# vccheng2001/DeepVCP-Pointcloud-Registration

Hardware: AMD Instinct MI355X
Metric: pairs/sec (full DeepVCP forward) at N=16384, K=64; rot/trans error vs ref (higher is better)
Workload: dtype f32

## Files before the change

### deepvcp-pointcloud-registration_amd/csrc/sa_mlp_mfma.hip

```cpp
#include "common.h"
#include "morton.h"

namespace dvcp {

typedef float f32x16 __attribute__((ext_vector_type(16)));
typedef __bf16 bf16x8 __attribute__((ext_vector_type(8)));

#ifndef DVCP_SA_SPLIT3
#define DVCP_SA_SPLIT3 1
#endif
#ifndef DVCP_SA_PACK16
#define DVCP_SA_PACK16 1
#endif

struct Split3 {
  bf16x8 p0, p1, p2;
};
__device__ __forceinline__ Split3 split3(const float (&x)[8]) {
  Split3 s;
#pragma unroll
  for (int j = 0; j < 8; ++j) {
    const __bf16 b0 = static_cast<__bf16>(x[j]);
    const float r1 = x[j] - static_cast<float>(b0);
    const __bf16 b1 = static_cast<__bf16>(r1);
    const float r2 = r1 - static_cast<float>(b1);
    s.p0[j] = b0;
    s.p1[j] = b1;
    s.p2[j] = static_cast<__bf16>(r2);
  }
  return s;
}
__device__ __forceinline__ f32x16 mfma_split3(const Split3& a, const bf16x8& b0, const bf16x8& b1, const bf16x8& b2,
                                             f32x16 acc) {
  acc = __builtin_amdgcn_mfma_f32_32x32x16_bf16(a.p2, b0, acc, 0, 0, 0);
  acc = __builtin_amdgcn_mfma_f32_32x32x16_bf16(a.p1, b1, acc, 0, 0, 0);
  acc = __builtin_amdgcn_mfma_f32_32x32x16_bf16(a.p0, b2, acc, 0, 0, 0);
  acc = __builtin_amdgcn_mfma_f32_32x32x16_bf16(a.p1, b0, acc, 0, 0, 0);
  acc = __builtin_amdgcn_mfma_f32_32x32x16_bf16(a.p0, b1, acc, 0, 0, 0);
  return __builtin_amdgcn_mfma_f32_32x32x16_bf16(a.p0, b0, acc, 0, 0, 0);
}

constexpr int kMfmaWaves = 4;

template <int D, int C1, int C2>
struct SaMfmaShape {
  static constexpr int C0 = 3 + D;
  static constexpr int KS = 3 + D / 2;
  static constexpr int MT = C1 / 32;
  static constexpr int CT = C2 / 32;
  static constexpr int K2 = MT * 16;
  static constexpr int KB = MT * 2;
  static_assert(D % 8 == 0 && C1 % 32 == 0 && C2 % 32 == 0, "MFMA tiling");
};

template <int D, int C1, int C2, bool PRE>
struct SaMfmaLds {
  using S = SaMfmaShape<D, C1, C2>;
  float w1[PRE ? 1 : S::MT][S::KS][64];
  float wx[S::MT][2][64];
#if DVCP_SA_SPLIT3
  bf16x8 w2s[S::CT][S::KB][3][64];
#else
  float w2[S::CT][S::K2][64];
#endif
  float b1[S::MT][2][16];
  float s1[S::MT][2][16];
  float t1[S::MT][2][16];
};

template <int D>
__device__ __forceinline__ int sa_in_channel(int s, int h) {
  if (s < 3) return h == 0 ? s : -1;
  return 3 + h * (D / 2) + (s - 3);
}

__device__ __forceinline__ int acc_row(int r, int h) { return (r & 3) + 8 * (r >> 2) + 4 * h; }

template <int D, int C1>
__global__ __launch_bounds__(256) void sa_pre_mfma_kernel(const float* __restrict__ feat, int64_t fb, int64_t fn, int N,
                                                          int B, const float* __restrict__ params,
                                                          float* __restrict__ U, const int64_t* __restrict__ rows,
                                                          int Nf) {
  constexpr int C0 = 3 + D, MT = C1 / 32, KS = D / 2;
  static_assert(D % 8 == 0 && C1 % 32 == 0, "MFMA tiling");
  __shared__ float wf[MT][KS][64];
  __shared__ float bias[C1];
  const float* W1 = params;
  const float* pb1 = W1 + C1 * C0;
  const float* ps1 = pb1 + C1;
  const float* pt1 = ps1 + C1;
  for (int i = threadIdx.x; i < MT * KS * 64; i += blockDim.x) {
    const int l = i % 64, s = (i / 64) % KS, mt = i / (64 * KS), o = 32 * mt + (l & 31);
    wf[mt][s][l] = W1[o * C0 + 3 + s + (l >> 5) * (D / 2)] * ps1[o];
  }
  for (int c = threadIdx.x; c < C1; c += blockDim.x)
    bias[c] = static_cast<float>(static_cast<double>(pb1[c]) * ps1[c] + static_cast<double>(pt1[c]));
  __syncthreads();
  const int lane = threadIdx.x & 63, h = lane >> 5, r32 = lane & 31;
  const int64_t total = static_cast<int64_t>(B) * N;
  const int64_t ntiles = (total + 31) / 32;
  for (int64_t t = static_cast<int64_t>(blockIdx.x) * 4 + (threadIdx.x >> 6); t < ntiles;
       t += static_cast<int64_t>(gridDim.x) * 4) {
    const int64_t i = t * 32 + r32;
    const int64_t ic = i < total ? i : total - 1;
    const int b = static_cast<int>(ic / N), n = static_cast<int>(ic % N);
    int64_t src = n;
    if (rows) {
      const int64_t r = rows[ic];
      src = r < 0 ? 0 : (r >= Nf ? Nf - 1 : r);
    }
    const float4* fr = reinterpret_cast<const float4*>(feat + b * fb + src * fn + h * (D / 2));
    float x[KS];
#pragma unroll
    for (int v = 0; v < KS / 4; ++v) {
      const float4 q = fr[v];
      x[4 * v] = q.x;
      x[4 * v + 1] = q.y;
      x[4 * v + 2] = q.z;
      x[4 * v + 3] = q.w;
    }
    int zo = 0;
    asm volatile("" : "+v"(zo));
    f32x16 acc[MT];
#pragma unroll
    for (int mt = 0; mt < MT; ++mt) {
      const float bc = bias[32 * mt + r32 + zo];
#pragma unroll
      for (int r = 0; r < 16; ++r) acc[mt][r] = bc;
    }
#pragma unroll
    for (int s = 0; s < KS; ++s)
#pragma unroll
      for (int mt = 0; mt < MT; ++mt)
        acc[mt] = __builtin_amdgcn_mfma_f32_32x32x2f32(x[s], wf[mt][s][lane + zo], acc[mt], 0, 0, 0);
#pragma unroll
    for (int r = 0; r < 16; ++r) {
      const int64_t ip = t * 32 + acc_row(r, h);
      if (ip < total)
#pragma unroll
        for (int mt = 0; mt < MT; ++mt) U[ip * C1 + 32 * mt + r32] = acc[mt][r];
    }
  }
}

template <typename T>
__global__ __launch_bounds__(kBuildThreads) void sa_order_kernel(PointsView<T> ctr, int S, int32_t* __restrict__ order) {
  __shared__ uint32_t bins[kSortBins];
  __shared__ uint32_t wsum[16];
  __shared__ float red[2][3][16];
  const int b = blockIdx.x;
  auto get = [&](int i, float (&v)[3]) {
#pragma unroll
    for (int a = 0; a < 3; ++a) v[a] = static_cast<float>(ctr.at(b, a, i));
  };
  float lo[3], hi[3];
  block_bbox(S, get, lo, hi, red);
  int32_t* o = order + static_cast<int64_t>(b) * S;
  morton_sort(S, get, [&](int pos, int i, const float (&)[3]) { o[pos] = i; }, lo, hi, bins, wsum);
}

template <typename T, int D, int C1, int C2, bool PRE, bool PACK = false>
__global__ __launch_bounds__(kMfmaWaves * kWave) __attribute__((amdgpu_waves_per_eu(3))) void sa_mlp_mfma_kernel(
    PointsView<T> pts, PointsView<T> ctr, int S, int B, const float* __restrict__ feat, int64_t fb, int64_t fn,
    const int32_t* __restrict__ count, const int32_t* __restrict__ list, int nsample,
    const float* __restrict__ params, const float* __restrict__ U, int64_t ub, const int32_t* __restrict__ order,
    float* __restrict__ out, int xcd) {
  using Sh = SaMfmaShape<D, C1, C2>;
  constexpr int C0 = Sh::C0, KS = Sh::KS, MT = Sh::MT, CT = Sh::CT;
  __shared__ SaMfmaLds<D, C1, C2, PRE> L;
  const int tid = threadIdx.x, lane = tid & 63, wave = tid >> 6, h = lane >> 5, r32 = lane & 31;

  const float* W1 = params;
  const float* pb1 = W1 + C1 * C0;
  const float* ps1 = pb1 + C1;
  const float* pt1 = ps1 + C1;
  const float* W2 = pt1 + C1;
  const float* pb2 = W2 + C2 * C1;
  const float* ps2 = pb2 + C2;
  const float* pt2 = ps2 + C2;
  if (!PRE)
    for (int i = tid; i < MT * KS * 64; i += blockDim.x) {
      const int l = i % 64, s = (i / 64) % KS, mt = i / (64 * KS);
      const int ch = sa_in_channel<D>(s, l >> 5);
      L.w1[mt][s][l] = ch < 0 ? 0.0f : W1[(32 * mt + (l & 31)) * C0 + ch];
    }
  if (PRE)
    for (int i = tid; i < MT * 2 * 64; i += blockDim.x) {
      const int l = i % 64, s = (i / 64) % 2, mt = i / 128;
      const int ch = s == 0 ? (l >> 5) : ((l >> 5) == 0 ? 2 : -1);
      L.wx[mt][s][l] = ch < 0 ? 0.0f : W1[(32 * mt + (l & 31)) * C0 + ch] * ps1[32 * mt + (l & 31)];
    }
#if DVCP_SA_SPLIT3
  for (int i = tid; i < CT * Sh::KB * 64; i += blockDim.x) {
    const int l = i % 64, s = (i / 64) % Sh::KB, ct = i / (64 * Sh::KB);
    const int o = 32 * ct + (l & 31);
    float w[8];
#pragma unroll
    for (int j = 0; j < 8; ++j)
      w[j] = W2[o * C1 + 32 * (s / 2) + acc_row(8 * (s % 2) + j, l >> 5)] * (PRE ? ps2[o] : 1.0f);
    const Split3 ws = split3(w);
    L.w2s[ct][s][0][l] = ws.p0;
    L.w2s[ct][s][1][l] = ws.p1;
    L.w2s[ct][s][2][l] = ws.p2;
  }
#else
  for (int i = tid; i < CT * Sh::K2 * 64; i += blockDim.x) {
    const int l = i % 64, kk = (i / 64) % Sh::K2, ct = i / (64 * Sh::K2);
    const int mt = kk / 16, r = kk % 16;
    L.w2[ct][kk][l] = W2[(32 * ct + (l & 31)) * C1 + 32 * mt + acc_row(r, l >> 5)] * (PRE ? ps2[32 * ct + (l & 31)] : 1.0f);
  }
#endif
  for (int i = tid; i < MT * 32; i += blockDim.x) {
    const int r = i % 16, hh = (i / 16) % 2, mt = i / 32;
    const int c = 32 * mt + acc_row(r, hh);
    L.b1[mt][hh][r] = pb1[c];
    L.s1[mt][hh][r] = ps1[c];
    L.t1[mt][hh][r] = pt1[c];
  }
  float b2[CT], s2[CT], t2[CT];
#pragma unroll
  for (int ct = 0; ct < CT; ++ct) {
    b2[ct] = pb2[32 * ct + r32];
    s2[ct] = ps2[32 * ct + r32];
    t2[ct] = pt2[32 * ct + r32];
    if (PRE) b2[ct] = static_cast<float>(static_cast<double>(b2[ct]) * s2[ct] + static_cast<double>(t2[ct]));
  }
  __syncthreads();

  int64_t total, q0, qs;
  int xo = 0;
  if (xcd) {
    xo = static_cast<int>(blockIdx.x) & 7;
    total = static_cast<int64_t>((B - xo + 7) / 8) * S;
    q0 = static_cast<int64_t>(blockIdx.x >> 3) * kMfmaWaves + wave;
    qs = static_cast<int64_t>(gridDim.x >> 3) * kMfmaWaves;
  } else {
    total = static_cast<int64_t>(B) * S;
    q0 = static_cast<int64_t>(blockIdx.x) * kMfmaWaves + wave;
    qs = static_cast<int64_t>(gridDim.x) * kMfmaWaves;
  }
  auto lane_bcast = [](auto v, int j) {
    if constexpr (sizeof(v) == 8) {
      const int64_t u = __builtin_bit_cast(int64_t, v);
      const int lo = __builtin_amdgcn_readlane(static_cast<int>(u & 0xFFFFFFFF), j);
      const int hi = __builtin_amdgcn_readlane(static_cast<int>(u >> 32), j);
      return __builtin_bit_cast(decltype(v), (static_cast<int64_t>(hi) << 32) | static_cast<uint32_t>(lo));
    } else {
      return __builtin_bit_cast(decltype(v), __builtin_amdgcn_readlane(__builtin_bit_cast(int, v), j));
    }
  };
  for (int64_t qc = q0; qc < total; qc += 64 * qs) {
    const int64_t qm = qc + lane * qs;
    int m_b = 0, m_rows = 0;
    int64_t m_fc = 0;
    T m_cx = T(0), m_cy = T(0), m_cz = T(0);
    if (qm < total) {
      const int64_t q = xcd ? (xo + 8 * (qm / S)) * static_cast<int64_t>(S) + qm % S : qm;
      m_b = static_cast<int>(q / S);
      const int c = order ? order[q] : static_cast<int>(q % S);
      m_fc = static_cast<int64_t>(m_b) * S + c;
      const int r = count[m_fc];
      m_rows = r < 1 ? 0 : (r > nsample ? nsample : r);
      ctr.load3(m_b, c, m_cx, m_cy, m_cz);
    }
    const int ncen = static_cast<int>(min<int64_t>(64, (total - qc + qs - 1) / qs));
    auto list_entry = [&](int j, int n0) {
      const int64_t fcj = lane_bcast(m_fc, j);
      const int rj = lane_bcast(m_rows, j);
      const int row = n0 + r32;
      return rj == 0 ? 0 : list[fcj * nsample + (row < rj ? row : 0)];
    };
    constexpr bool BZ = PRE && DVCP_SA_SPLIT3;
    if constexpr (PACK) {
      static_assert(!PACK || (PRE && DVCP_SA_SPLIT3), "row packing runs on the split-3 pre-pass path");
      int js = 0, hs = 0;
      auto nh_of = [&](int jj) { return max(1, (lane_bcast(m_rows, jj) + 15) >> 4); };
      int nhj = ncen > 0 ? nh_of(0) : 0;
      int runj = -1;
      float run[CT];
#pragma unroll
      for (int ct = 0; ct < CT; ++ct) run[ct] = 0.0f;
      auto flush = [&]() {
        const int64_t fcr = lane_bcast(m_fc, runj);
        const bool empty = lane_bcast(m_rows, runj) == 0;
#pragma unroll
        for (int ct = 0; ct < CT; ++ct)
          if (h == 0) out[fcr * C2 + 32 * ct + r32] = empty ? 0.0f : fmaxf(run[ct] + b2[ct], 0.0f);
      };
      auto fold = [&](int jj, const float (&m)[CT]) {
        if (jj != runj) {
          if (runj >= 0) flush();
          runj = jj;
#pragma unroll
          for (int ct = 0; ct < CT; ++ct) run[ct] = m[ct];
        } else {
#pragma unroll
          for (int ct = 0; ct < CT; ++ct) run[ct] = fmaxf(run[ct], m[ct]);
        }
      };
      while (js < ncen) {
        const int jA = js, hA = hs;
        if (++hs >= nhj) {
          hs = 0;
          if (++js < ncen) nhj = nh_of(js);
        }
        const bool hasB = js < ncen;
        const int jB = hasB ? js : jA, hB = hasB ? hs : hA;
        if (hasB && ++hs >= nhj) {
          hs = 0;
          if (++js < ncen) nhj = nh_of(js);
        }
        int zo = 0;
        asm volatile("" : "+v"(zo));
        const bool sB = r32 >= 16;
        const int b = sB ? lane_bcast(m_b, jB) : lane_bcast(m_b, jA);
        const int64_t fc = sB ? lane_bcast(m_fc, jB) : lane_bcast(m_fc, jA);
        const int rows = sB ? lane_bcast(m_rows, jB) : lane_bcast(m_rows, jA);
        const T cx = sB ? lane_bcast(m_cx, jB) : lane_bcast(m_cx, jA);
        const T cy = sB ? lane_bcast(m_cy, jB) : lane_bcast(m_cy, jA);
        const T cz = sB ? lane_bcast(m_cz, jB) : lane_bcast(m_cz, jA);
        const int row = 16 * (sB ? hB : hA) + (r32 & 15);
        const int n = rows == 0 ? 0 : list[fc * nsample + (row < rows ? row : 0)];
        f32x16 acc1[MT];
        const float4* ur = reinterpret_cast<const float4*>(U + b * ub + static_cast<int64_t>(n) * C1 + 4 * h);
#pragma unroll
        for (int mt = 0; mt < MT; ++mt)
#pragma unroll
          for (int i = 0; i < 4; ++i) {
            const float4 u = ur[8 * mt + 2 * i];
            acc1[mt][4 * i] = u.x;
            acc1[mt][4 * i + 1] = u.y;
            acc1[mt][4 * i + 2] = u.z;
            acc1[mt][4 * i + 3] = u.w;
          }
        T px, py, pz;
        pts.load3(b, n, px, py, pz);
        const float dx = static_cast<float>(px - cx);
        const float dy = static_cast<float>(py - cy);
        const float dz = static_cast<float>(pz - cz);
        const float x0 = h == 0 ? dx : dy, x1 = h == 0 ? dz : 0.0f;
#pragma unroll
        for (int mt = 0; mt < MT; ++mt) {
          acc1[mt] = __builtin_amdgcn_mfma_f32_32x32x2f32(L.wx[mt][0][lane + zo], x0, acc1[mt], 0, 0, 0);
          acc1[mt] = __builtin_amdgcn_mfma_f32_32x32x2f32(L.wx[mt][1][lane + zo], x1, acc1[mt], 0, 0, 0);
#pragma unroll
          for (int r = 0; r < 16; ++r) acc1[mt][r] = acc1[mt][r] > 0.0f ? acc1[mt][r] : 0.0f;
        }
        f32x16 acc2[CT];
#pragma unroll
        for (int ct = 0; ct < CT; ++ct)
#pragma unroll
          for (int r = 0; r < 16; ++r) acc2[ct][r] = 0.0f;
#pragma unroll
        for (int st = 0; st < Sh::KB; ++st) {
          float x[8];
#pragma unroll
          for (int jj = 0; jj < 8; ++jj) x[jj] = acc1[st / 2][8 * (st % 2) + jj];
          const Split3 a = split3(x);
#pragma unroll
          for (int ct = 0; ct < CT; ++ct)
            acc2[ct] = mfma_split3(a, L.w2s[ct][st][0][lane + zo], L.w2s[ct][st][1][lane + zo],
                                   L.w2s[ct][st][2][lane + zo], acc2[ct]);
        }
        float mA[CT], mB[CT];
#pragma unroll
        for (int ct = 0; ct < CT; ++ct) {
          float a0 = acc2[ct][0], a1 = acc2[ct][8];
#pragma unroll
          for (int r = 1; r < 8; ++r) {
            a0 = fmaxf(a0, acc2[ct][r]);
            a1 = fmaxf(a1, acc2[ct][8 + r]);
          }
          mA[ct] = fmaxf(a0, __shfl_xor(a0, 32, kWave));
          mB[ct] = fmaxf(a1, __shfl_xor(a1, 32, kWave));
        }
        fold(jA, mA);
        if (hasB) fold(jB, mB);
      }
      if (runj >= 0) flush();
      continue;
    }
    const uint64_t live_c = __ballot(lane < ncen && m_rows > 0);
    auto next_live = [&](int j) {
      const uint64_t m = j >= 63 ? 0ull : (live_c & (~0ull << (j + 1)));
      return m ? static_cast<int>(__builtin_ctzll(m)) : 64;
    };
    int n_next = 0;
    {
      const int j0 = (live_c & 1ull) ? 0 : next_live(0);
      if (j0 < ncen) n_next = list_entry(j0, 0);
    }
  for (int j = 0; j < ncen; ++j) {
    const int b = lane_bcast(m_b, j);
    const int64_t fc = lane_bcast(m_fc, j);
    const int rows = lane_bcast(m_rows, j);
    const T cx = lane_bcast(m_cx, j), cy = lane_bcast(m_cy, j), cz = lane_bcast(m_cz, j);
    float mx[CT];
#pragma unroll
    for (int ct = 0; ct < CT; ++ct) mx[ct] = BZ ? -__builtin_huge_valf() : 0.0f;

    for (int n0 = 0; n0 < rows; n0 += 32) {
      int zo = 0;
      asm volatile("" : "+v"(zo));
      const int n = n_next;
      if (n0 + 32 < rows)
        n_next = list_entry(j, n0 + 32);
      else if (next_live(j) < ncen)
        n_next = list_entry(next_live(j), 0);
      f32x16 acc1[MT];
      if constexpr (PRE) {
        const float4* ur = reinterpret_cast<const float4*>(U + b * ub + static_cast<int64_t>(n) * C1 + 4 * h);
#pragma unroll
        for (int mt = 0; mt < MT; ++mt)
#pragma unroll
          for (int i = 0; i < 4; ++i) {
            const float4 u = ur[8 * mt + 2 * i];
            acc1[mt][4 * i] = u.x;
            acc1[mt][4 * i + 1] = u.y;
            acc1[mt][4 * i + 2] = u.z;
            acc1[mt][4 * i + 3] = u.w;
          }
        T px, py, pz;
        pts.load3(b, n, px, py, pz);
        const float dx = static_cast<float>(px - cx);
        const float dy = static_cast<float>(py - cy);
        const float dz = static_cast<float>(pz - cz);
        const float x0 = h == 0 ? dx : dy, x1 = h == 0 ? dz : 0.0f;
#pragma unroll
        for (int mt = 0; mt < MT; ++mt) {
          acc1[mt] = __builtin_amdgcn_mfma_f32_32x32x2f32(L.wx[mt][0][lane + zo], x0, acc1[mt], 0, 0, 0);
          acc1[mt] = __builtin_amdgcn_mfma_f32_32x32x2f32(L.wx[mt][1][lane + zo], x1, acc1[mt], 0, 0, 0);
        }
      } else {
        float x[KS];
        if (h == 0) {
          x[0] = static_cast<float>(pts.at(b, 0, n) - cx);
          x[1] = static_cast<float>(pts.at(b, 1, n) - cy);
          x[2] = static_cast<float>(pts.at(b, 2, n) - cz);
        } else {
          x[0] = x[1] = x[2] = 0.0f;
        }
        const float4* fr = reinterpret_cast<const float4*>(feat + b * fb + static_cast<int64_t>(n) * fn + h * (D / 2));
#pragma unroll
        for (int v = 0; v < D / 8; ++v) {
          const float4 f = fr[v];
          x[3 + 4 * v] = f.x;
          x[4 + 4 * v] = f.y;
          x[5 + 4 * v] = f.z;
          x[6 + 4 * v] = f.w;
        }
#pragma unroll
        for (int mt = 0; mt < MT; ++mt)
#pragma unroll
          for (int r = 0; r < 16; ++r) acc1[mt][r] = L.b1[mt][h][r + zo];
#pragma unroll
        for (int s = 0; s < KS; ++s)
#pragma unroll
          for (int mt = 0; mt < MT; ++mt)
            acc1[mt] = __builtin_amdgcn_mfma_f32_32x32x2f32(L.w1[mt][s][lane + zo], x[s], acc1[mt], 0, 0, 0);
      }
#pragma unroll
      for (int mt = 0; mt < MT; ++mt)
#pragma unroll
        for (int r = 0; r < 16; ++r) {
          const float v = PRE ? acc1[mt][r] : acc1[mt][r] * L.s1[mt][h][r + zo] + L.t1[mt][h][r + zo];
          acc1[mt][r] = v > 0.0f ? v : 0.0f;
        }
      f32x16 acc2[CT];
#pragma unroll
      for (int ct = 0; ct < CT; ++ct)
#pragma unroll
        for (int r = 0; r < 16; ++r) acc2[ct][r] = BZ ? 0.0f : b2[ct];
#if DVCP_SA_SPLIT3
#pragma unroll
      for (int s = 0; s < Sh::KB; ++s) {
        float x[8];
#pragma unroll
        for (int j = 0; j < 8; ++j) x[j] = acc1[s / 2][8 * (s % 2) + j];
        const Split3 a = split3(x);
#pragma unroll
        for (int ct = 0; ct < CT; ++ct)
          acc2[ct] = mfma_split3(a, L.w2s[ct][s][0][lane + zo], L.w2s[ct][s][1][lane + zo], L.w2s[ct][s][2][lane + zo],
                                 acc2[ct]);
      }
#else
#pragma unroll
      for (int mt = 0; mt < MT; ++mt)
#pragma unroll
        for (int r = 0; r < 16; ++r)
#pragma unroll
          for (int ct = 0; ct < CT; ++ct)
            acc2[ct] = __builtin_amdgcn_mfma_f32_32x32x2f32(acc1[mt][r], L.w2[ct][mt * 16 + r][lane + zo], acc2[ct], 0, 0, 0);
#endif
#pragma unroll
      for (int ct = 0; ct < CT; ++ct)
#pragma unroll
        for (int r = 0; r < 16; ++r) {
          if (PRE) {
            mx[ct] = fmaxf(mx[ct], acc2[ct][r]);
          } else {
            const float v = acc2[ct][r] * s2[ct] + t2[ct];
            mx[ct] = fmaxf(mx[ct], v > 0.0f ? v : 0.0f);
          }
        }
    }
#pragma unroll
    for (int ct = 0; ct < CT; ++ct) {
      float m = fmaxf(mx[ct], __shfl_xor(mx[ct], 32, kWave));
      if (BZ) m = fmaxf(m + b2[ct], 0.0f);
      if (h == 0) out[fc * C2 + 32 * ct + r32] = m;
    }
  }
  }
}

struct Sa3Lds {
  float w1[3][64];
  bf16x8 w2[3][64];
  bf16x8 w3[3][64];
  float b1[2][8];
  float b2[2][8];
};

template <typename T, typename FT, int D>
__global__ __launch_bounds__(kMfmaWaves * kWave) void sa3_mfma_kernel(
    PointsView<T> pts, PointsView<T> ctr, int S, int B, const FT* __restrict__ feat, int64_t fb, int64_t fd, int64_t fn,
    const int32_t* __restrict__ count, const int32_t* __restrict__ list, int nsample, const float* __restrict__ params,
    float* __restrict__ out, int xcd) {
  constexpr int C0 = 3 + D, C1 = 16, C2 = 16, C3 = 32;
  constexpr int KS = (C0 + 1) / 2;
  static_assert(D == 0 || D == 3, "sa1 tables");
  __shared__ Sa3Lds L;
  const int tid = threadIdx.x, lane = tid & 63, wave = tid >> 6, h = lane >> 5, r32 = lane & 31;
  const float* W1 = params;
  const float* pb1 = W1 + C1 * C0;
  const float* ps1 = pb1 + C1;
  const float* pt1 = ps1 + C1;
  const float* W2 = pt1 + C1;
  const float* pb2 = W2 + C2 * C1;
  const float* ps2 = pb2 + C2;
  const float* pt2 = ps2 + C2;
  const float* W3 = pt2 + C2;
  const float* pb3 = W3 + C3 * C2;
  const float* ps3 = pb3 + C3;
  const float* pt3 = ps3 + C3;
  auto fold_bias = [](float b, float s, float t) {
    return static_cast<float>(static_cast<double>(b) * s + static_cast<double>(t));
  };
  for (int i = tid; i < KS * 64; i += blockDim.x) {
    const int l = i % 64, s = i / 64, o = l & 31, c = 2 * s + (l >> 5);
    L.w1[s][l] = (o < C1 && c < C0) ? W1[o * C0 + c] * ps1[o] : 0.0f;
  }
  if (tid < 64) {
    const int o = tid & 31, kh = tid >> 5;
    float a[8], w[8];
#pragma unroll
    for (int r = 0; r < 8; ++r) {
      a[r] = o < C2 ? W2[o * C1 + acc_row(r, kh)] * ps2[o] : 0.0f;
      w[r] = W3[o * C2 + acc_row(r, kh)] * ps3[o];
    }
    const Split3 sa = split3(a), sw = split3(w);
    L.w2[0][tid] = sa.p0;
    L.w2[1][tid] = sa.p1;
    L.w2[2][tid] = sa.p2;
    L.w3[0][tid] = sw.p0;
    L.w3[1][tid] = sw.p1;
    L.w3[2][tid] = sw.p2;
  } else if (tid < 80) {
    const int kh = (tid - 64) >> 3, r = tid & 7, c = acc_row(r, kh);
    L.b1[kh][r] = fold_bias(pb1[c], ps1[c], pt1[c]);
    L.b2[kh][r] = fold_bias(pb2[c], ps2[c], pt2[c]);
  }
  const float b3 = fold_bias(pb3[r32], ps3[r32], pt3[r32]);
  __syncthreads();

  int64_t total, q0, qs;
  int xo = 0;
  if (xcd) {
    xo = static_cast<int>(blockIdx.x) & 7;
    total = static_cast<int64_t>((B - xo + 7) / 8) * S;
    q0 = static_cast<int64_t>(blockIdx.x >> 3) * kMfmaWaves + wave;
    qs = static_cast<int64_t>(gridDim.x >> 3) * kMfmaWaves;
  } else {
    total = static_cast<int64_t>(B) * S;
    q0 = static_cast<int64_t>(blockIdx.x) * kMfmaWaves + wave;
    qs = static_cast<int64_t>(gridDim.x) * kMfmaWaves;
  }
  auto lane_bcast = [](auto v, int j) {
    if constexpr (sizeof(v) == 8) {
      const int64_t u = __builtin_bit_cast(int64_t, v);
      const int lo = __builtin_amdgcn_readlane(static_cast<int>(u & 0xFFFFFFFF), j);
      const int hi = __builtin_amdgcn_readlane(static_cast<int>(u >> 32), j);
      return __builtin_bit_cast(decltype(v), (static_cast<int64_t>(hi) << 32) | static_cast<uint32_t>(lo));
    } else {
      return __builtin_bit_cast(decltype(v), __builtin_amdgcn_readlane(__builtin_bit_cast(int, v), j));
    }
  };
  for (int64_t qc = q0; qc < total; qc += 64 * qs) {
    const int64_t qm = qc + lane * qs;
    int m_b = 0, m_rows = 0;
    int64_t m_fc = 0;
    T m_cx = T(0), m_cy = T(0), m_cz = T(0);
    if (qm < total) {
      const int64_t q = xcd ? (xo + 8 * (qm / S)) * static_cast<int64_t>(S) + qm % S : qm;
      m_b = static_cast<int>(q / S);
      m_fc = q;
      const int r = count[q];
      m_rows = r < 0 ? 0 : (r > nsample ? nsample : r);
      const int c = static_cast<int>(q % S);
      ctr.load3(m_b, c, m_cx, m_cy, m_cz);
    }
    const int ncen = static_cast<int>(min<int64_t>(64, (total - qc + qs - 1) / qs));
    int js = 0, hs = 0;
    auto nh_of = [&](int jj) { return max(1, (lane_bcast(m_rows, jj) + 15) >> 4); };
    int nhj = ncen > 0 ? nh_of(0) : 0;
    int runj = -1;
    float run = 0.0f;
    auto flush = [&]() {
      const int64_t fcr = lane_bcast(m_fc, runj);
      const bool empty = lane_bcast(m_rows, runj) == 0;
      if (h == 0) out[fcr * C3 + r32] = empty ? 0.0f : fmaxf(run + b3, 0.0f);
    };
    auto fold = [&](int jj, float m) {
      if (jj != runj) {
        if (runj >= 0) flush();
        runj = jj;
        run = m;
      } else {
        run = fmaxf(run, m);
      }
    };
    while (js < ncen) {
      const int jA = js, hA = hs;
      if (++hs >= nhj) {
        hs = 0;
        if (++js < ncen) nhj = nh_of(js);
      }
      const bool hasB = js < ncen;
      const int jB = hasB ? js : jA, hB = hasB ? hs : hA;
      if (hasB && ++hs >= nhj) {
        hs = 0;
        if (++js < ncen) nhj = nh_of(js);
      }
      int zo = 0;
      asm volatile("" : "+v"(zo));
      const bool sB = r32 >= 16;
      const int b = sB ? lane_bcast(m_b, jB) : lane_bcast(m_b, jA);
      const int64_t fc = sB ? lane_bcast(m_fc, jB) : lane_bcast(m_fc, jA);
      const int rows = sB ? lane_bcast(m_rows, jB) : lane_bcast(m_rows, jA);
      const T cx = sB ? lane_bcast(m_cx, jB) : lane_bcast(m_cx, jA);
      const T cy = sB ? lane_bcast(m_cy, jB) : lane_bcast(m_cy, jA);
      const T cz = sB ? lane_bcast(m_cz, jB) : lane_bcast(m_cz, jA);
      const int row = 16 * (sB ? hB : hA) + (r32 & 15);
      const int n = rows == 0 ? 0 : list[fc * nsample + (row < rows ? row : 0)];
      T px, py, pz;
      pts.load3(b, n, px, py, pz);
      const float dx = static_cast<float>(px - cx);
      const float dy = static_cast<float>(py - cy);
      const float dz = static_cast<float>(pz - cz);
      float x[KS];
      x[0] = h == 0 ? dx : dy;
      if constexpr (D == 0) {
        x[1] = h == 0 ? dz : 0.0f;
      } else {
        const FT* f = feat + b * fb + static_cast<int64_t>(n) * fn;
        x[1] = h == 0 ? dz : static_cast<float>(f[0]);
        x[2] = static_cast<float>(h == 0 ? f[fd] : f[2 * fd]);
      }
      f32x16 a1;
#pragma unroll
      for (int r = 0; r < 8; ++r) {
        a1[r] = L.b1[h][r + zo];
        a1[8 + r] = 0.0f;
      }
#pragma unroll
      for (int s = 0; s < KS; ++s) a1 = __builtin_amdgcn_mfma_f32_32x32x2f32(L.w1[s][lane + zo], x[s], a1, 0, 0, 0);
      float v[8];
#pragma unroll
      for (int r = 0; r < 8; ++r) v[r] = fmaxf(a1[r], 0.0f);
      const Split3 p1 = split3(v);
      f32x16 a2;
#pragma unroll
      for (int r = 0; r < 8; ++r) {
        a2[r] = L.b2[h][r + zo];
        a2[8 + r] = 0.0f;
      }
      const Split3 w2{L.w2[0][lane + zo], L.w2[1][lane + zo], L.w2[2][lane + zo]};
      a2 = mfma_split3(w2, p1.p0, p1.p1, p1.p2, a2);
#pragma unroll
      for (int r = 0; r < 8; ++r) v[r] = fmaxf(a2[r], 0.0f);
      const Split3 p2 = split3(v);
      f32x16 a3;
#pragma unroll
      for (int r = 0; r < 16; ++r) a3[r] = 0.0f;
      a3 = mfma_split3(p2, L.w3[0][lane + zo], L.w3[1][lane + zo], L.w3[2][lane + zo], a3);
      float mA = a3[0], mB = a3[8];
#pragma unroll
      for (int r = 1; r < 8; ++r) {
        mA = fmaxf(mA, a3[r]);
        mB = fmaxf(mB, a3[8 + r]);
      }
      mA = fmaxf(mA, __shfl_xor(mA, 32, kWave));
      mB = fmaxf(mB, __shfl_xor(mB, 32, kWave));
      fold(jA, mA);
      if (hasB) fold(jB, mB);
    }
    if (runj >= 0) flush();
  }
}

#ifndef DVCP_SA_GRID
#define DVCP_SA_GRID 4096
#endif
constexpr int kSaGrid = DVCP_SA_GRID;

template <typename T, typename FT, int D>
int launch_sa3_mfma(const void* xyz, int64_t sb, int64_t sc, int64_t sn, const void* c, int64_t cb, int64_t cc,
                    int64_t cn, int S, int B, const void* feat, int64_t fb, int64_t fd, int64_t fn, const int32_t* count,
                    const int32_t* list, int nsample, const float* params, float* out, hipStream_t st) {
  PointsView<T> pv{static_cast<const T*>(xyz), sb, sc, sn};
  PointsView<T> cv{static_cast<const T*>(c), cb, cc, cn};
  const int64_t centres = static_cast<int64_t>(B) * S;
  const int grid = static_cast<int>(centres < kSaGrid * kMfmaWaves ? (centres + kMfmaWaves - 1) / kMfmaWaves : kSaGrid);
  const int xcd = B % 8 == 0 && grid % 8 == 0 ? 1 : 0;
  hipLaunchKernelGGL((sa3_mfma_kernel<T, FT, D>), dim3(grid), dim3(kMfmaWaves * kWave), 0, st, pv, cv, S, B,
                     static_cast<const FT*>(feat), fb, fd, fn, count, list, nsample, params, out, xcd);
  return launch_status("dvcp_sa_group_mlp(mfma3)");
}

#define DVCP_SA3_MFMA_INST(T, FT, D)                                                                              \
  template int launch_sa3_mfma<T, FT, D>(const void*, int64_t, int64_t, int64_t, const void*, int64_t, int64_t,  \
                                         int64_t, int, int, const void*, int64_t, int64_t, int64_t, const int32_t*, \
                                         const int32_t*, int, const float*, float*, hipStream_t);
DVCP_SA3_MFMA_INST(float, float, 0)
DVCP_SA3_MFMA_INST(float, double, 0)
DVCP_SA3_MFMA_INST(double, float, 0)
DVCP_SA3_MFMA_INST(double, double, 0)
DVCP_SA3_MFMA_INST(float, float, 3)
DVCP_SA3_MFMA_INST(float, double, 3)
DVCP_SA3_MFMA_INST(double, float, 3)
DVCP_SA3_MFMA_INST(double, double, 3)
#undef DVCP_SA3_MFMA_INST

template <typename T, int D, int C1, int C2>
int launch_sa_mfma(const void* xyz, int64_t sb, int64_t sc, int64_t sn, int N, const void* c, int64_t cb, int64_t cc,
                   int64_t cn, int S, int B, const float* feat, int64_t fb, int64_t fn, const int32_t* count,
                   const int32_t* list, int nsample, const float* params, float* U, int32_t* order, float* out,
                   const int64_t* frows, int Nf, hipStream_t st) {
  PointsView<T> pv{static_cast<const T*>(xyz), sb, sc, sn};
  PointsView<T> cv{static_cast<const T*>(c), cb, cc, cn};
  const int64_t centres = static_cast<int64_t>(B) * S;
  const int grid = static_cast<int>(centres < kSaGrid * kMfmaWaves ? (centres + kMfmaWaves - 1) / kMfmaWaves : kSaGrid);
  const int xcd = B % 8 == 0 && grid % 8 == 0 ? 1 : 0;
  if (order)
    hipLaunchKernelGGL((sa_order_kernel<T>), dim3(B), dim3(kBuildThreads), 0, st, cv, S, order);
  if (U) {
    const int64_t rows = static_cast<int64_t>(B) * N;
    const int64_t wgs = (rows + 127) / 128;
    hipLaunchKernelGGL((sa_pre_mfma_kernel<D, C1>), dim3(static_cast<unsigned>(wgs < 2048 ? wgs : 2048)), dim3(256), 0,
                       st, feat, fb, fn, N, B, params, U, frows, Nf);
    if constexpr (DVCP_SA_PACK16 && DVCP_SA_SPLIT3 && D == 32)
      hipLaunchKernelGGL((sa_mlp_mfma_kernel<T, D, C1, C2, true, DVCP_SA_PACK16 && DVCP_SA_SPLIT3>), dim3(grid),
                         dim3(kMfmaWaves * kWave), 0, st, pv, cv, S, B, feat, fb, fn, count, list, nsample, params, U,
                         static_cast<int64_t>(N) * C1, order, out, xcd);
    else
      hipLaunchKernelGGL((sa_mlp_mfma_kernel<T, D, C1, C2, true>), dim3(grid), dim3(kMfmaWaves * kWave), 0, st, pv, cv,
                         S, B, feat, fb, fn, count, list, nsample, params, U, static_cast<int64_t>(N) * C1, order, out, xcd);
  } else {
    hipLaunchKernelGGL((sa_mlp_mfma_kernel<T, D, C1, C2, false>), dim3(grid), dim3(kMfmaWaves * kWave), 0, st, pv,
                       cv, S, B, feat, fb, fn, count, list, nsample, params, nullptr, 0, order, out, xcd);
  }
  return launch_status("dvcp_sa_group_mlp(mfma)");
}

#define DVCP_SA_MFMA_INST(T, D, C1, C2)                                                                          \
  template int launch_sa_mfma<T, D, C1, C2>(const void*, int64_t, int64_t, int64_t, int, const void*, int64_t,  \
                                            int64_t, int64_t, int, int, const float*, int64_t, int64_t,         \
                                            const int32_t*, const int32_t*, int, const float*, float*,          \
                                            int32_t*, float*, const int64_t*, int, hipStream_t);
DVCP_SA_MFMA_INST(float, 32, 32, 64)
DVCP_SA_MFMA_INST(double, 32, 32, 64)
DVCP_SA_MFMA_INST(float, 64, 64, 64)
DVCP_SA_MFMA_INST(double, 64, 64, 64)
#undef DVCP_SA_MFMA_INST

}
```

Baseline: 2523.

## Software-pipeline neighbor loads and interleave split-3 conversion with MFMA in SA kernel

Restructures the SA MLP MFMA kernel so the next tile's neighbor index is fetched one step ahead and its feature and point loads are issued before the current tile's math. It adds a layer-2 helper that computes the bf16 split-3 of the next k-step while the current k-step's MFMAs run, using sched_group_barrier hints to interleave VALU work with MFMA. The non-packed path is flattened into one loop over live center tiles, and empty centers are zero-filled up front. The sa3 kernel also gets a waves_per_eu(4) occupancy hint. The cost is more register pressure from prefetched operands and double-buffered split values, plus more complex control flow.

```diff
diff --git a/deepvcp-pointcloud-registration_amd/csrc/sa_mlp_mfma.hip b/deepvcp-pointcloud-registration_amd/csrc/sa_mlp_mfma.hip
--- a/deepvcp-pointcloud-registration_amd/csrc/sa_mlp_mfma.hip
+++ b/deepvcp-pointcloud-registration_amd/csrc/sa_mlp_mfma.hip
@@ -38,6 +38,78 @@
   acc = __builtin_amdgcn_mfma_f32_32x32x16_bf16(a.p1, b0, acc, 0, 0, 0);
   acc = __builtin_amdgcn_mfma_f32_32x32x16_bf16(a.p0, b1, acc, 0, 0, 0);
   return __builtin_amdgcn_mfma_f32_32x32x16_bf16(a.p0, b0, acc, 0, 0, 0);
+}
+
+constexpr int kSchedValu = 0x2, kSchedMfma = 0x8;
+
+template <int MT, int CT, bool IL>
+__device__ __forceinline__ void sa_layer2_split3(const f32x16 (&acc1)[MT], const bf16x8 (&w2s)[CT][2 * MT][3][64],
+                                                 int li, f32x16 (&acc2)[CT]) {
+  constexpr int KB = 2 * MT;
+  static_assert(CT % 2 == 0, "6 CT MFMAs per k-step in four equal runs");
+  constexpr int Q = 6 * CT / 4;
+  constexpr int VPG = (13 + Q - 1) / Q;
+  auto split_pair = [&](int s, int i, bf16x8 (&p)[3]) {
+#pragma unroll
+    for (int j = 2 * i; j < 2 * i + 2; ++j) {
+      const float v = acc1[s / 2][8 * (s % 2) + j];
+      const float x = v > 0.0f ? v : 0.0f;
+      const __bf16 b0 = static_cast<__bf16>(x);
+      const float r1 = x - static_cast<float>(b0);
+      const __bf16 b1 = static_cast<__bf16>(r1);
+      const float r2 = r1 - static_cast<float>(b1);
+      p[0][j] = b0;
+      p[1][j] = b1;
+      p[2][j] = static_cast<__bf16>(r2);
+    }
+  };
+  if constexpr (!IL) {
+#pragma unroll
+    for (int s = 0; s < KB; ++s) {
+      float x[8];
+#pragma unroll
+      for (int j = 0; j < 8; ++j) {
+        const float v = acc1[s / 2][8 * (s % 2) + j];
+        x[j] = v > 0.0f ? v : 0.0f;
+      }
+      const Split3 as = split3(x);
+#pragma unroll
+      for (int ct = 0; ct < CT; ++ct) acc2[ct] = mfma_split3(as, w2s[ct][s][0][li], w2s[ct][s][1][li], w2s[ct][s][2][li], acc2[ct]);
+    }
+    return;
+  }
+  bf16x8 a[3], an[3];
+#pragma unroll
+  for (int i = 0; i < 4; ++i) split_pair(0, i, a);
+#pragma unroll
+  for (int s = 0; s < KB; ++s) {
+    bf16x8 w[CT][3];
+#pragma unroll
+    for (int ct = 0; ct < CT; ++ct)
+#pragma unroll
+      for (int p = 0; p < 3; ++p) w[ct][p] = w2s[ct][s][p][li];
+#pragma unroll
+    for (int r = 0; r < 4; ++r) {
+      if (s + 1 < KB) split_pair(s + 1, r, an);
+#pragma unroll
+      for (int m = r * Q; m < (r + 1) * Q; ++m) {
+        const int pc = m / CT, ct = m % CT;
+        const int ia = pc == 0 ? 2 : (pc == 1 || pc == 3) ? 1 : 0;
+        const int ib = pc == 2 ? 2 : (pc == 1 || pc == 4) ? 1 : 0;
+        acc2[ct] = __builtin_amdgcn_mfma_f32_32x32x16_bf16(a[ia], w[ct][ib], acc2[ct], 0, 0, 0);
+      }
+      if (s + 1 < KB) {
+#pragma unroll
+        for (int g = 0; g < Q; ++g) {
+          __builtin_amdgcn_sched_group_barrier(kSchedMfma, 1, 0);
+          __builtin_amdgcn_sched_group_barrier(kSchedValu, VPG, 0);
+        }
+      }
+      __builtin_amdgcn_sched_barrier(0);
+    }
+#pragma unroll
+    for (int p = 0; p < 3; ++p) a[p] = an[p];
+  }
 }
 
 constexpr int kMfmaWaves = 4;
@@ -271,6 +343,62 @@
       return rj == 0 ? 0 : list[fcj * nsample + (row < rj ? row : 0)];
     };
     constexpr bool BZ = PRE && DVCP_SA_SPLIT3;
+    constexpr int NV = PRE ? 4 * MT : D / 8;
+    struct Ops {
+      float4 v[NV];
+      T px, py, pz;
+    };
+    auto load_ops = [&](int b, int n, Ops& o) {
+      const float4* r = PRE ? reinterpret_cast<const float4*>(U + b * ub + static_cast<int64_t>(n) * C1 + 4 * h)
+                            : reinterpret_cast<const float4*>(feat + b * fb + static_cast<int64_t>(n) * fn + h * (D / 2));
+#pragma unroll
+      for (int i = 0; i < NV; ++i) o.v[i] = r[PRE ? 2 * i : i];
+      pts.load3(b, n, o.px, o.py, o.pz);
+    };
+    auto layer1 = [&](const Ops& o, T cx, T cy, T cz, int zo, f32x16 (&acc1)[MT]) {
+      const float dx = static_cast<float>(o.px - cx);
+      const float dy = static_cast<float>(o.py - cy);
+      const float dz = static_cast<float>(o.pz - cz);
+      if constexpr (PRE) {
+#pragma unroll
+        for (int mt = 0; mt < MT; ++mt)
+#pragma unroll
+          for (int i = 0; i < 4; ++i) {
+            const float4 u = o.v[4 * mt + i];
+            acc1[mt][4 * i] = u.x;
+            acc1[mt][4 * i + 1] = u.y;
+            acc1[mt][4 * i + 2] = u.z;
+            acc1[mt][4 * i + 3] = u.w;
+          }
+        const float x0 = h == 0 ? dx : dy, x1 = h == 0 ? dz : 0.0f;
+#pragma unroll
+        for (int mt = 0; mt < MT; ++mt) {
+          acc1[mt] = __builtin_amdgcn_mfma_f32_32x32x2f32(L.wx[mt][0][lane + zo], x0, acc1[mt], 0, 0, 0);
+          acc1[mt] = __builtin_amdgcn_mfma_f32_32x32x2f32(L.wx[mt][1][lane + zo], x1, acc1[mt], 0, 0, 0);
+        }
+      } else {
+        float x[KS];
+        x[0] = h == 0 ? dx : 0.0f;
+        x[1] = h == 0 ? dy : 0.0f;
+        x[2] = h == 0 ? dz : 0.0f;
+#pragma unroll
+        for (int v = 0; v < D / 8; ++v) {
+          x[3 + 4 * v] = o.v[v].x;
+          x[4 + 4 * v] = o.v[v].y;
+          x[5 + 4 * v] = o.v[v].z;
+          x[6 + 4 * v] = o.v[v].w;
+        }
+#pragma unroll
+        for (int mt = 0; mt < MT; ++mt)
+#pragma unroll
+          for (int r = 0; r < 16; ++r) acc1[mt][r] = L.b1[mt][h][r + zo];
+#pragma unroll
+        for (int s = 0; s < KS; ++s)
+#pragma unroll
+          for (int mt = 0; mt < MT; ++mt)
+            acc1[mt] = __builtin_amdgcn_mfma_f32_32x32x2f32(L.w1[mt][s][lane + zo], x[s], acc1[mt], 0, 0, 0);
+      }
+    };
     if constexpr (PACK) {
       static_assert(!PACK || (PRE && DVCP_SA_SPLIT3), "row packing runs on the split-3 pre-pass path");
       int js = 0, hs = 0;
@@ -298,70 +426,58 @@
           for (int ct = 0; ct < CT; ++ct) run[ct] = fmaxf(run[ct], m[ct]);
         }
       };
-      while (js < ncen) {
-        const int jA = js, hA = hs;
+      struct HalfPair {
+        int jA, hA, jB, hB;
+        bool hasB;
+      };
+      auto take_pair = [&](HalfPair& p) {
+        if (js >= ncen) return false;
+        p.jA = js;
+        p.hA = hs;
         if (++hs >= nhj) {
           hs = 0;
           if (++js < ncen) nhj = nh_of(js);
         }
-        const bool hasB = js < ncen;
-        const int jB = hasB ? js : jA, hB = hasB ? hs : hA;
-        if (hasB && ++hs >= nhj) {
+        p.hasB = js < ncen;
+        p.jB = p.hasB ? js : p.jA;
+        p.hB = p.hasB ? hs : p.hA;
+        if (p.hasB && ++hs >= nhj) {
           hs = 0;
           if (++js < ncen) nhj = nh_of(js);
         }
+        return true;
+      };
+      const bool sB = r32 >= 16;
+      auto pair_entry = [&](const HalfPair& p, int& b) {
+        b = sB ? lane_bcast(m_b, p.jB) : lane_bcast(m_b, p.jA);
+        const int64_t fc = sB ? lane_bcast(m_fc, p.jB) : lane_bcast(m_fc, p.jA);
+        const int rows = sB ? lane_bcast(m_rows, p.jB) : lane_bcast(m_rows, p.jA);
+        const int row = 16 * (sB ? p.hB : p.hA) + (r32 & 15);
+        return rows == 0 ? 0 : list[fc * nsample + (row < rows ? row : 0)];
+      };
+      HalfPair cur{}, nxt{};
+      bool vc = take_pair(cur);
+      int b_nx = 0, n_nx = 0;
+      if (vc) n_nx = pair_entry(cur, b_nx);
+      while (vc) {
+        nxt = cur;
+        const bool vn = take_pair(nxt);
         int zo = 0;
         asm volatile("" : "+v"(zo));
-        const bool sB = r32 >= 16;
-        const int b = sB ? lane_bcast(m_b, jB) : lane_bcast(m_b, jA);
-        const int64_t fc = sB ? lane_bcast(m_fc, jB) : lane_bcast(m_fc, jA);
-        const int rows = sB ? lane_bcast(m_rows, jB) : lane_bcast(m_rows, jA);
-        const T cx = sB ? lane_bcast(m_cx, jB) : lane_bcast(m_cx, jA);
-        const T cy = sB ? lane_bcast(m_cy, jB) : lane_bcast(m_cy, jA);
-        const T cz = sB ? lane_bcast(m_cz, jB) : lane_bcast(m_cz, jA);
-        const int row = 16 * (sB ? hB : hA) + (r32 & 15);
-        const int n = rows == 0 ? 0 : list[fc * nsample + (row < rows ? row : 0)];
+        const T cx = sB ? lane_bcast(m_cx, cur.jB) : lane_bcast(m_cx, cur.jA);
+        const T cy = sB ? lane_bcast(m_cy, cur.jB) : lane_bcast(m_cy, cur.jA);
+        const T cz = sB ? lane_bcast(m_cz, cur.jB) : lane_bcast(m_cz, cur.jA);
+        Ops ops;
+        load_ops(b_nx, n_nx, ops);
+        n_nx = pair_entry(nxt, b_nx);
         f32x16 acc1[MT];
-        const float4* ur = reinterpret_cast<const float4*>(U + b * ub + static_cast<int64_t>(n) * C1 + 4 * h);
-#pragma unroll
-        for (int mt = 0; mt < MT; ++mt)
-#pragma unroll
-          for (int i = 0; i < 4; ++i) {
-            const float4 u = ur[8 * mt + 2 * i];
-            acc1[mt][4 * i] = u.x;
-            acc1[mt][4 * i + 1] = u.y;
-            acc1[mt][4 * i + 2] = u.z;
-            acc1[mt][4 * i + 3] = u.w;
-          }
-        T px, py, pz;
-        pts.load3(b, n, px, py, pz);
-        const float dx = static_cast<float>(px - cx);
-        const float dy = static_cast<float>(py - cy);
-        const float dz = static_cast<float>(pz - cz);
-        const float x0 = h == 0 ? dx : dy, x1 = h == 0 ? dz : 0.0f;
-#pragma unroll
-        for (int mt = 0; mt < MT; ++mt) {
-          acc1[mt] = __builtin_amdgcn_mfma_f32_32x32x2f32(L.wx[mt][0][lane + zo], x0, acc1[mt], 0, 0, 0);
-          acc1[mt] = __builtin_amdgcn_mfma_f32_32x32x2f32(L.wx[mt][1][lane + zo], x1, acc1[mt], 0, 0, 0);
-#pragma unroll
-          for (int r = 0; r < 16; ++r) acc1[mt][r] = acc1[mt][r] > 0.0f ? acc1[mt][r] : 0.0f;
-        }
+        layer1(ops, cx, cy, cz, zo, acc1);
         f32x16 acc2[CT];
 #pragma unroll
         for (int ct = 0; ct < CT; ++ct)
 #pragma unroll
           for (int r = 0; r < 16; ++r) acc2[ct][r] = 0.0f;
-#pragma unroll
-        for (int st = 0; st < Sh::KB; ++st) {
-          float x[8];
-#pragma unroll
-          for (int jj = 0; jj < 8; ++jj) x[jj] = acc1[st / 2][8 * (st % 2) + jj];
-          const Split3 a = split3(x);
-#pragma unroll
-          for (int ct = 0; ct < CT; ++ct)
-            acc2[ct] = mfma_split3(a, L.w2s[ct][st][0][lane + zo], L.w2s[ct][st][1][lane + zo],
-                                   L.w2s[ct][st][2][lane + zo], acc2[ct]);
-        }
+        sa_layer2_split3<MT, CT, PRE>(acc1, L.w2s, lane + zo, acc2);
         float mA[CT], mB[CT];
 #pragma unroll
         for (int ct = 0; ct < CT; ++ct) {
@@ -374,91 +490,62 @@
           mA[ct] = fmaxf(a0, __shfl_xor(a0, 32, kWave));
           mB[ct] = fmaxf(a1, __shfl_xor(a1, 32, kWave));
         }
-        fold(jA, mA);
-        if (hasB) fold(jB, mB);
+        fold(cur.jA, mA);
+        if (cur.hasB) fold(cur.jB, mB);
+        cur = nxt;
+        vc = vn;
       }
       if (runj >= 0) flush();
       continue;
     }
     const uint64_t live_c = __ballot(lane < ncen && m_rows > 0);
+    if (lane < ncen && m_rows == 0)
+      for (int c = 0; c < C2; ++c) out[m_fc * C2 + c] = 0.0f;
     auto next_live = [&](int j) {
       const uint64_t m = j >= 63 ? 0ull : (live_c & (~0ull << (j + 1)));
       return m ? static_cast<int>(__builtin_ctzll(m)) : 64;
     };
-    int n_next = 0;
-    {
-      const int j0 = (live_c & 1ull) ? 0 : next_live(0);
-      if (j0 < ncen) n_next = list_entry(j0, 0);
-    }
-  for (int j = 0; j < ncen; ++j) {
-    const int b = lane_bcast(m_b, j);
-    const int64_t fc = lane_bcast(m_fc, j);
-    const int rows = lane_bcast(m_rows, j);
-    const T cx = lane_bcast(m_cx, j), cy = lane_bcast(m_cy, j), cz = lane_bcast(m_cz, j);
+    auto next_tile = [&](int& j, int& n0) {
+      if (n0 + 32 < lane_bcast(m_rows, j)) {
+        n0 += 32;
+        return true;
+      }
+      const int jn = next_live(j);
+      if (jn >= 64) return false;
+      j = jn;
+      n0 = 0;
+      return true;
+    };
+    if (live_c == 0) continue;
+    int jc = static_cast<int>(__builtin_ctzll(live_c)), nc = 0;
+    int n_nx = list_entry(jc, nc);
     float mx[CT];
 #pragma unroll
     for (int ct = 0; ct < CT; ++ct) mx[ct] = BZ ? -__builtin_huge_valf() : 0.0f;
-
-    for (int n0 = 0; n0 < rows; n0 += 32) {
+    for (bool vc = true; vc;) {
+      int jn = jc, nn = nc;
+      const bool vn = next_tile(jn, nn);
       int zo = 0;
       asm volatile("" : "+v"(zo));
-      const int n = n_next;
-      if (n0 + 32 < rows)
-        n_next = list_entry(j, n0 + 32);
-      else if (next_live(j) < ncen)
-        n_next = list_entry(next_live(j), 0);
+      Ops ops;
+      load_ops(lane_bcast(m_b, jc), n_nx, ops);
+      n_nx = list_entry(jn, nn);
       f32x16 acc1[MT];
-      if constexpr (PRE) {
-        const float4* ur = reinterpret_cast<const float4*>(U + b * ub + static_cast<int64_t>(n) * C1 + 4 * h);
+      layer1(ops, lane_bcast(m_cx, jc), lane_bcast(m_cy, jc), lane_bcast(m_cz, jc), zo, acc1);
+      f32x16 acc2[CT];
+#pragma unroll
+      for (int ct = 0; ct < CT; ++ct)
+#pragma unroll
+        for (int r = 0; r < 16; ++r) acc2[ct][r] = BZ ? 0.0f : b2[ct];
+#if DVCP_SA_SPLIT3
+      if constexpr (!PRE) {
 #pragma unroll
         for (int mt = 0; mt < MT; ++mt)
 #pragma unroll
-          for (int i = 0; i < 4; ++i) {
-            const float4 u = ur[8 * mt + 2 * i];
-            acc1[mt][4 * i] = u.x;
-            acc1[mt][4 * i + 1] = u.y;
-            acc1[mt][4 * i + 2] = u.z;
-            acc1[mt][4 * i + 3] = u.w;
-          }
-        T px, py, pz;
-        pts.load3(b, n, px, py, pz);
-        const float dx = static_cast<float>(px - cx);
-        const float dy = static_cast<float>(py - cy);
-        const float dz = static_cast<float>(pz - cz);
-        const float x0 = h == 0 ? dx : dy, x1 = h == 0 ? dz : 0.0f;
-#pragma unroll
-        for (int mt = 0; mt < MT; ++mt) {
-          acc1[mt] = __builtin_amdgcn_mfma_f32_32x32x2f32(L.wx[mt][0][lane + zo], x0, acc1[mt], 0, 0, 0);
-          acc1[mt] = __builtin_amdgcn_mfma_f32_32x32x2f32(L.wx[mt][1][lane + zo], x1, acc1[mt], 0, 0, 0);
-        }
-      } else {
-        float x[KS];
-        if (h == 0) {
-          x[0] = static_cast<float>(pts.at(b, 0, n) - cx);
-          x[1] = static_cast<float>(pts.at(b, 1, n) - cy);
-          x[2] = static_cast<float>(pts.at(b, 2, n) - cz);
-        } else {
-          x[0] = x[1] = x[2] = 0.0f;
-        }
-        const float4* fr = reinterpret_cast<const float4*>(feat + b * fb + static_cast<int64_t>(n) * fn + h * (D / 2));
-#pragma unroll
-        for (int v = 0; v < D / 8; ++v) {
-          const float4 f = fr[v];
-          x[3 + 4 * v] = f.x;
-          x[4 + 4 * v] = f.y;
-          x[5 + 4 * v] = f.z;
-          x[6 + 4 * v] = f.w;
-        }
-#pragma unroll
-        for (int mt = 0; mt < MT; ++mt)
-#pragma unroll
-          for (int r = 0; r < 16; ++r) acc1[mt][r] = L.b1[mt][h][r + zo];
-#pragma unroll
-        for (int s = 0; s < KS; ++s)
-#pragma unroll
-          for (int mt = 0; mt < MT; ++mt)
-            acc1[mt] = __builtin_amdgcn_mfma_f32_32x32x2f32(L.w1[mt][s][lane + zo], x[s], acc1[mt], 0, 0, 0);
-      }
+          for (int r = 0; r < 16; ++r) acc1[mt][r] = acc1[mt][r] * L.s1[mt][h][r + zo] + L.t1[mt][h][r + zo];
+      }
+      sa_layer2_split3<MT, CT, PRE>(acc1, L.w2s, lane + zo, acc2);
+#else
 #pragma unroll
       for (int mt = 0; mt < MT; ++mt)
 #pragma unroll
@@ -466,24 +553,6 @@
           const float v = PRE ? acc1[mt][r] : acc1[mt][r] * L.s1[mt][h][r + zo] + L.t1[mt][h][r + zo];
           acc1[mt][r] = v > 0.0f ? v : 0.0f;
         }
-      f32x16 acc2[CT];
-#pragma unroll
-      for (int ct = 0; ct < CT; ++ct)
-#pragma unroll
-        for (int r = 0; r < 16; ++r) acc2[ct][r] = BZ ? 0.0f : b2[ct];
-#if DVCP_SA_SPLIT3
-#pragma unroll
-      for (int s = 0; s < Sh::KB; ++s) {
-        float x[8];
-#pragma unroll
-        for (int j = 0; j < 8; ++j) x[j] = acc1[s / 2][8 * (s % 2) + j];
-        const Split3 a = split3(x);
-#pragma unroll
-        for (int ct = 0; ct < CT; ++ct)
-          acc2[ct] = mfma_split3(a, L.w2s[ct][s][0][lane + zo], L.w2s[ct][s][1][lane + zo], L.w2s[ct][s][2][lane + zo],
-                                 acc2[ct]);
-      }
-#else
 #pragma unroll
       for (int mt = 0; mt < MT; ++mt)
 #pragma unroll
@@ -503,14 +572,20 @@
             mx[ct] = fmaxf(mx[ct], v > 0.0f ? v : 0.0f);
           }
         }
-    }
-#pragma unroll
-    for (int ct = 0; ct < CT; ++ct) {
-      float m = fmaxf(mx[ct], __shfl_xor(mx[ct], 32, kWave));
-      if (BZ) m = fmaxf(m + b2[ct], 0.0f);
-      if (h == 0) out[fc * C2 + 32 * ct + r32] = m;
-    }
-  }
+      if (!vn || jn != jc) {
+        const int64_t fc = lane_bcast(m_fc, jc);
+#pragma unroll
+        for (int ct = 0; ct < CT; ++ct) {
+          float m = fmaxf(mx[ct], __shfl_xor(mx[ct], 32, kWave));
+          if (BZ) m = fmaxf(m + b2[ct], 0.0f);
+          if (h == 0) out[fc * C2 + 32 * ct + r32] = m;
+          mx[ct] = BZ ? -__builtin_huge_valf() : 0.0f;
+        }
+      }
+      vc = vn;
+      jc = jn;
+      nc = nn;
+    }
   }
 }
 
@@ -523,7 +598,7 @@
 };
 
 template <typename T, typename FT, int D>
-__global__ __launch_bounds__(kMfmaWaves * kWave) void sa3_mfma_kernel(
+__global__ __launch_bounds__(kMfmaWaves * kWave) __attribute__((amdgpu_waves_per_eu(4))) void sa3_mfma_kernel(
     PointsView<T> pts, PointsView<T> ctr, int S, int B, const FT* __restrict__ feat, int64_t fb, int64_t fd, int64_t fn,
     const int32_t* __restrict__ count, const int32_t* __restrict__ list, int nsample, const float* __restrict__ params,
     float* __restrict__ out, int xcd) {
```

New measurement: 2527, median of 2. Within noise of the previous version (+0.2%).
